# darskkaa/NTIRE-2026-Light-Field-Image-Super-Resolution-Challenge---Track-2-Efficiency

Measured on AMD Instinct MI355X. Metric: 5x5 x4-SR LF patches/sec (32^2->128^2), DistgSSR inference, higher is better.
Workload: dtype f32 (EPI branch stage 1 / 2 and fuse.0: fp32 operands as three exact bf16 terms on the bf16 MFMA pipe, six products, fp32 accumulation -- error against fp64 not above the fp32-MFMA kernels', tests/test_gpu_b3_accuracy.py; 3x3 convs, angular branch, init, head: fp32 MFMA)

## Files before the change

ntire-2026-light-field-image-super-resolution-challenge---track-2-efficiency_amd/csrc/distg_tail.hip:

```cpp
#include "lfsr_internal.h"

namespace {

typedef float f32x4t __attribute__((ext_vector_type(4)));
typedef unsigned u32x4t __attribute__((ext_vector_type(4)));

constexpr int DT_WAVES = 8;
constexpr int DT_FPLANE = 64 * 160;
constexpr int DT_FBYTES = 3 * DT_FPLANE * 2;
constexpr int DT_ESLOTS = 3 * 4 * 160;
constexpr int DT_EBYTES = DT_ESLOTS * 16;
constexpr int DT_AFLOATS = 25 * 16 * 16;
constexpr int DT_ABYTES = DT_AFLOATS * 4;
constexpr int DT_CROW = 84;
constexpr int DT_CBYTES = DT_WAVES * 16 * DT_CROW * 4;
constexpr int DT_SMEM = DT_FBYTES + DT_EBYTES + DT_ABYTES + DT_CBYTES;

struct DistgTailArgs {
  const float* S; int s_stride; int s_choff; int s_bytes;
  const float* TA; int ta_bytes;
  const float* TH; const float* TV; int te_bytes;
  const float* WA2;
  const uint4* WE2p;
  const float* WF;
  float* Y; int y_stride; int y_choff; int y_bytes;
  int B, H, W;
  float slope;
};

__device__ __forceinline__ void dt_split8(const f32x4t lo, const f32x4t hi, u32x4t& p0, u32x4t& p1, u32x4t& p2) {
  const float a[8] = {lo.x, lo.y, lo.z, lo.w, hi.x, hi.y, hi.z, hi.w};
#pragma unroll
  for (int j = 0; j < 4; ++j) { unsigned t0, t1, t2; lfsr_split_pair(a[2 * j], a[2 * j + 1], t0, t1, t2); p0[j] = t0; p1[j] = t1; p2[j] = t2; }
}

__device__ __forceinline__ void dt_mfma(f32x4t& c, const u32x4t a, const u32x4t b) {
  asm volatile("v_mfma_f32_16x16x32_bf16 %0, %1, %2, %0" : "+v"(c) : "v"(a), "v"(b));
}

__device__ __forceinline__ void dt_six2(f32x4t& c0, const u32x4t (&a)[3], const u32x4t (&x)[3], f32x4t& c1, const u32x4t (&b)[3], const u32x4t (&y)[3]) {
  dt_mfma(c0, a[2], x[0]); dt_mfma(c1, b[2], y[0]);
  dt_mfma(c0, a[0], x[2]); dt_mfma(c1, b[0], y[2]);
  dt_mfma(c0, a[1], x[1]); dt_mfma(c1, b[1], y[1]);
  dt_mfma(c0, a[1], x[0]); dt_mfma(c1, b[1], y[0]);
  dt_mfma(c0, a[0], x[1]); dt_mfma(c1, b[0], y[1]);
  dt_mfma(c0, a[0], x[0]); dt_mfma(c1, b[0], y[0]);
}

__global__ __launch_bounds__(512) void k_distg_tail(DistgTailArgs p) {
  extern __shared__ __attribute__((aligned(16))) unsigned char smem_raw[];
  unsigned short* const sF = reinterpret_cast<unsigned short*>(smem_raw);
  unsigned char* const sE = smem_raw + DT_FBYTES;
  float* const sA = reinterpret_cast<float*>(smem_raw + DT_FBYTES + DT_EBYTES);
  float* const sC = reinterpret_cast<float*>(smem_raw + DT_FBYTES + DT_EBYTES + DT_ABYTES);
  constexpr int A = 5, AA = 25;
  constexpr int EOOB = (int)0x80000000u;
  const int tid = threadIdx.x, lane = tid & 63, wave = tid >> 6;
  const int l15 = lane & 15, g = lane >> 4;
  const int HW = p.H * p.W, M = p.B * HW;
  const int ntiles = (M + 15) / 16;

  for (int i = tid; i < 64 * 20; i += 512) {
    const int r = i / 20, c = i - r * 20;
    const bool ok = c * 8 < 144;
    const float* src = p.WF + r * 144 + (ok ? c * 8 : 0);
    f32x4t lo = *reinterpret_cast<const f32x4t*>(src), hi = *reinterpret_cast<const f32x4t*>(src + 4);
    if (!ok) { lo = f32x4t{0.f, 0.f, 0.f, 0.f}; hi = lo; }
    u32x4t w0, w1, w2;
    dt_split8(lo, hi, w0, w1, w2);
    const int slot = (c * 64 + r) * 8;
    *reinterpret_cast<u32x4t*>(sF + 0 * DT_FPLANE + slot) = w0;
    *reinterpret_cast<u32x4t*>(sF + 1 * DT_FPLANE + slot) = w1;
    *reinterpret_cast<u32x4t*>(sF + 2 * DT_FPLANE + slot) = w2;
  }
  for (int i = tid; i < DT_ESLOTS; i += 512) reinterpret_cast<uint4*>(sE)[i] = p.WE2p[i];
  for (int i = tid; i < DT_AFLOATS / 4; i += 512) reinterpret_cast<float4*>(sA)[i] = reinterpret_cast<const float4*>(p.WA2)[i];
  __syncthreads();

  const __amdgpu_buffer_rsrc_t rsS = __builtin_amdgcn_make_buffer_rsrc(const_cast<float*>(p.S), 0, p.s_bytes, 0x00020000);
  const __amdgpu_buffer_rsrc_t rsA = __builtin_amdgcn_make_buffer_rsrc(const_cast<float*>(p.TA), 0, p.ta_bytes, 0x00020000);
  const __amdgpu_buffer_rsrc_t rsH = __builtin_amdgcn_make_buffer_rsrc(const_cast<float*>(p.TH), 0, p.te_bytes, 0x00020000);
  const __amdgpu_buffer_rsrc_t rsV = __builtin_amdgcn_make_buffer_rsrc(const_cast<float*>(p.TV), 0, p.te_bytes, 0x00020000);
  const __amdgpu_buffer_rsrc_t rsY = __builtin_amdgcn_make_buffer_rsrc(p.Y, 0, p.y_bytes, 0x00020000);
  float* const st = sC + wave * 16 * DT_CROW;
  const unsigned char* const wE = sE + (g * 160 + l15) * 16;
  const unsigned short* const wF = sF + (g * 64 + l15) * 8;
  const float* const bA = sA + l15 * 16 + 4 * g;

  for (int tile = (int)blockIdx.x * DT_WAVES + wave; tile < ntiles; tile += (int)gridDim.x * DT_WAVES) {
    const int m = tile * 16 + l15;
    const bool ok = m < M;
    const int mb = ok ? m / HW : 0, myx = ok ? m - mb * HW : 0;
    auto tro = [&](int q) { return ok ? (((mb * A + q) * HW + myx) * 32 + 4 * g) * 4 : EOOB; };
    auto pixo = [&](int view) { return ok ? ((mb * AA + view) * HW + myx) : -1; };
    const f32x4t a2 = __builtin_bit_cast(f32x4t, __builtin_amdgcn_raw_buffer_load_b128(rsA, ok ? (m * 16 + 4 * g) * 4 : EOOB, 0, 0));

    f32x4t sr0[2][2], sr1[2][2], vr0[2], vr1[2], hr[2];
    auto load_view = [&](int view, f32x4t (&sr)[2][2], f32x4t (&vr)[2]) {
      const int pix = pixo(view);
      const int so = pix >= 0 ? (pix * p.s_stride + p.s_choff + 8 * g) * 4 : EOOB;
#pragma unroll
      for (int s = 0; s < 2; ++s)
#pragma unroll
        for (int e = 0; e < 2; ++e) sr[s][e] = __builtin_bit_cast(f32x4t, __builtin_amdgcn_raw_buffer_load_b128(rsS, so == EOOB ? EOOB : so + (32 * s + 4 * e) * 4, 0, 0));
      const int vo = tro(view % A);
      vr[0] = __builtin_bit_cast(f32x4t, __builtin_amdgcn_raw_buffer_load_b128(rsV, vo, 0, 0));
      vr[1] = __builtin_bit_cast(f32x4t, __builtin_amdgcn_raw_buffer_load_b128(rsV, vo == EOOB ? EOOB : vo + 64, 0, 0));
    };
    auto load_h = [&](int u) {
      const int ho = tro(u);
      hr[0] = __builtin_bit_cast(f32x4t, __builtin_amdgcn_raw_buffer_load_b128(rsH, ho, 0, 0));
      hr[1] = __builtin_bit_cast(f32x4t, __builtin_amdgcn_raw_buffer_load_b128(rsH, ho == EOOB ? EOOB : ho + 64, 0, 0));
    };
    load_h(0);
    load_view(0, sr0, vr0);
    u32x4t hp[3];

    auto body = [&](int view, f32x4t (&sr)[2][2], f32x4t (&vr)[2], f32x4t (&srn)[2][2], f32x4t (&vrn)[2]) {
      const int u = view / A, v = view - A * u;
      if (view + 1 < AA) load_view(view + 1, srn, vrn);
      if (v == 0) dt_split8(hr[0], hr[1], hp[0], hp[1], hp[2]);
      if (v == A - 1 && u + 1 < A) load_h(u + 1);

      {
        const float4 b = *reinterpret_cast<const float4*>(bA + view * 256);
        f32x4t o = {0.f, 0.f, 0.f, 0.f};
        o = __builtin_amdgcn_mfma_f32_16x16x4f32(a2.x, b.x, o, 0, 0, 0);
        o = __builtin_amdgcn_mfma_f32_16x16x4f32(a2.y, b.y, o, 0, 0, 0);
        o = __builtin_amdgcn_mfma_f32_16x16x4f32(a2.z, b.z, o, 0, 0, 0);
        o = __builtin_amdgcn_mfma_f32_16x16x4f32(a2.w, b.w, o, 0, 0, 0);
#pragma unroll
        for (int r = 0; r < 4; ++r) {
          float z = o[r];
          z = z >= 0.f ? z : z * p.slope;
          st[(4 * g + r) * DT_CROW + l15] = z;
        }
      }

      {
        u32x4t vp[3];
        dt_split8(vr[0], vr[1], vp[0], vp[1], vp[2]);
        asm volatile("s_nop 4" : "+v"(hp[0]), "+v"(hp[1]), "+v"(hp[2]), "+v"(vp[0]), "+v"(vp[1]), "+v"(vp[2]));
        f32x4t e[2][2];
#pragma unroll
        for (int i = 0; i < 2; ++i) { e[i][0] = f32x4t{0.f, 0.f, 0.f, 0.f}; e[i][1] = e[i][0]; }
        asm volatile("s_nop 1" : "+v"(e[0][0]), "+v"(e[0][1]), "+v"(e[1][0]), "+v"(e[1][1]));
#pragma unroll
        for (int h = 0; h < 2; ++h) {
          u32x4t aH[3], aV[3];
#pragma unroll
          for (int pl = 0; pl < 3; ++pl) {
            aH[pl] = *reinterpret_cast<const u32x4t*>(wE + ((pl * 4) * 160 + 16 * (2 * v + h)) * 16);
            aV[pl] = *reinterpret_cast<const u32x4t*>(wE + ((pl * 4) * 160 + 16 * (2 * u + h)) * 16);
          }
          dt_six2(e[0][h], aH, hp, e[1][h], aV, vp);
        }
        asm volatile("s_nop 15\n\ts_nop 15" : "+v"(e[0][0]), "+v"(e[0][1]), "+v"(e[1][0]), "+v"(e[1][1]));
#pragma unroll
        for (int i = 0; i < 2; ++i)
#pragma unroll
          for (int h = 0; h < 2; ++h) {
            f32x4t z = e[i][h];
#pragma unroll
            for (int r = 0; r < 4; ++r) z[r] = fmaxf(z[r], z[r] * p.slope);
            *reinterpret_cast<f32x4t*>(st + l15 * DT_CROW + 16 + 32 * i + 16 * h + 4 * g) = z;
          }
      }
      __builtin_amdgcn_wave_barrier();

      u32x4t x0[5], x1[5], x2[5];
#pragma unroll
      for (int s = 0; s < 2; ++s) dt_split8(sr[s][0], sr[s][1], x0[s], x1[s], x2[s]);
#pragma unroll
      for (int s = 2; s < 5; ++s) {
        const float* cp = st + l15 * DT_CROW + 32 * (s - 2) + 8 * g;
        f32x4t lo = *reinterpret_cast<const f32x4t*>(cp), hi = *reinterpret_cast<const f32x4t*>(cp + 4);
        if (s == 4 && g >= 2) { lo = f32x4t{0.f, 0.f, 0.f, 0.f}; hi = lo; }
        dt_split8(lo, hi, x0[s], x1[s], x2[s]);
      }
      __builtin_amdgcn_wave_barrier();
      f32x4t acc[4];
#pragma unroll
      for (int t = 0; t < 4; ++t) acc[t] = f32x4t{0.f, 0.f, 0.f, 0.f};
#pragma unroll
      for (int s = 0; s < 5; ++s) asm volatile("s_nop 4" : "+v"(x0[s]), "+v"(x1[s]), "+v"(x2[s]));
      asm volatile("s_nop 1" : "+v"(acc[0]), "+v"(acc[1]), "+v"(acc[2]), "+v"(acc[3]));
#pragma unroll
      for (int s = 0; s < 5; ++s) {
        const u32x4t xs[3] = {x0[s], x1[s], x2[s]};
#pragma unroll
        for (int t = 0; t < 4; t += 2) {
          u32x4t wa[3], wb[3];
#pragma unroll
          for (int pl = 0; pl < 3; ++pl) {
            wa[pl] = *reinterpret_cast<const u32x4t*>(wF + pl * DT_FPLANE + (4 * s * 64 + t * 16) * 8);
            wb[pl] = *reinterpret_cast<const u32x4t*>(wF + pl * DT_FPLANE + (4 * s * 64 + (t + 1) * 16) * 8);
          }
          dt_six2(acc[t], wa, xs, acc[t + 1], wb, xs);
        }
      }
      asm volatile("s_nop 15\n\ts_nop 15" : "+v"(acc[0]), "+v"(acc[1]), "+v"(acc[2]), "+v"(acc[3]));
      const int pix = pixo(view);
      const int yo = pix >= 0 ? (pix * p.y_stride + p.y_choff + 4 * g) * 4 : EOOB;
#pragma unroll
      for (int t = 0; t < 4; ++t) {
        f32x4t z = acc[t];
#pragma unroll
        for (int r = 0; r < 4; ++r) z[r] = z[r] >= 0.f ? z[r] : z[r] * p.slope;
        __builtin_amdgcn_raw_buffer_store_b128(__builtin_bit_cast(u32x4t, z), rsY, yo == EOOB ? EOOB : yo + 64 * t, 0, 0);
        asm volatile("s_nop 1" : "+v"(z));
      }
    };
#pragma unroll 1
    for (int view = 0; view < AA - 1; view += 2) {
      body(view, sr0, vr0, sr1, vr1);
      body(view + 1, sr1, vr1, sr0, vr0);
    }
    body(AA - 1, sr0, vr0, sr1, vr1);
  }
}

}

int lfsr_distg_tail_launch(const float* spa, int spa_stride, int spa_choff, const float* t_a, const float* t_h, const float* t_v, const float* wa2_packed,
                           const float* we2_planes, const float* wf_packed, float* y, int y_stride, int y_choff, int B, int A, int h, int w, float slope,
                           hipStream_t st) {
  if (A != 5 || B <= 0 || h <= 0 || w <= 0 || !spa || !t_a || !t_h || !t_v || !wa2_packed || !we2_planes || !wf_packed || !y) return LFSR_E_ARG;
  if ((spa_stride | spa_choff | y_stride | y_choff) & 3 || spa_stride < spa_choff + 64 || y_stride < y_choff + 64) return LFSR_E_ARG;
  if (((uintptr_t)spa | (uintptr_t)t_a | (uintptr_t)t_h | (uintptr_t)t_v | (uintptr_t)wa2_packed | (uintptr_t)we2_planes | (uintptr_t)wf_packed | (uintptr_t)y) & 15)
    return LFSR_E_ARG;
  if (!(slope >= 0.f && slope <= 1.f)) return LFSR_E_ARG;
  const long long npix = (long long)B * A * A * h * w;
  if (npix * spa_stride * 4 >= (1LL << 31) || npix * y_stride * 4 >= (1LL << 31) || (long long)B * A * h * w * 32 * 4 >= (1LL << 31)) return LFSR_E_ARG;
  static std::atomic<bool> attr_set[64];
  static std::atomic<int> cus[64];
  int dev = 0;
  if (hipGetDevice(&dev) != hipSuccess || dev < 0 || dev >= 64) return LFSR_E_ARG;
  if (!attr_set[dev]) {
    hipError_t e = hipFuncSetAttribute(reinterpret_cast<const void*>(k_distg_tail), hipFuncAttributeMaxDynamicSharedMemorySize, DT_SMEM);
    if (e != hipSuccess) return LFSR_HIP_ERR(e);
    int v = 0;
    cus[dev] = (hipDeviceGetAttribute(&v, hipDeviceAttributeMultiprocessorCount, dev) == hipSuccess && v > 0) ? v : 256;
    attr_set[dev] = true;
  }
  DistgTailArgs p{};
  p.S = spa; p.s_stride = spa_stride; p.s_choff = spa_choff; p.s_bytes = (int)(npix * spa_stride * 4);
  p.TA = t_a; p.ta_bytes = (int)((long long)B * h * w * 16 * 4);
  p.TH = t_h; p.TV = t_v; p.te_bytes = (int)((long long)B * A * h * w * 32 * 4);
  p.WA2 = wa2_packed; p.WE2p = reinterpret_cast<const uint4*>(we2_planes); p.WF = wf_packed;
  p.Y = y; p.y_stride = y_stride; p.y_choff = y_choff; p.y_bytes = (int)(npix * y_stride * 4);
  p.B = B; p.H = h; p.W = w; p.slope = slope;
  const long long ntiles = ((long long)B * h * w + 15) / 16;
  long long grid = (ntiles + DT_WAVES - 1) / DT_WAVES;
  if (grid > cus[dev]) grid = cus[dev];
  hipLaunchKernelGGL(k_distg_tail, dim3((unsigned)grid), dim3(DT_WAVES * 64), DT_SMEM, st, p);
  LFSR_CHECK_LAUNCH();
  return LFSR_OK;
}

bool lfsr_distg_tail_ok(int A, int h, int w, const float* x, int x_stride, int x_choff, const float* t_h, const float* t_v) {
  if (A != 5 || h <= 0 || w <= 0 || h > 32 || w > 32 || !lfsr_ang_fused_ok(A) || !lfsr_epi_use_b3()) return false;
  const char* rsel = lfsr_sel("LFSR_ROWGEMM");
  const char* asel = lfsr_sel("LFSR_ANG");
  if ((rsel && (rsel[0] == 'f' || rsel[0] == '1')) || lfsr_sel("LFSR_NO_ROWGEMM") || (asel && asel[0] == 'g')) return false;
  if ((x_stride | x_choff) & 3 || x_stride < x_choff + 64 || (((uintptr_t)x | (uintptr_t)t_h | (uintptr_t)t_v) & 15)) return false;
  return true;
}

extern "C" int lfsr_distg_branch_tail_fwd(const float* x, int x_stride, int x_choff, const float* spa, int spa_stride, int spa_choff,
                                          const float* w_ang0, const float* w_ang2, const float* w_epi0, const float* w_epi2, const float* w_fuse0,
                                          float* t_a, float* t_h, float* t_v, float* y, int y_stride, int y_choff, int B, int A, int h, int w, float slope,
                                          void* stream) {
  LfsrOpTimer op_t("distg_tail", B, h * w, lfsr_stream(stream));
  if (!x || !spa || !w_ang0 || !w_ang2 || !w_epi0 || !w_epi2 || !w_fuse0 || !t_a || !t_h || !t_v || !y || B <= 0) return LFSR_E_ARG;
  if (!lfsr_distg_tail_ok(A, h, w, x, x_stride, x_choff, t_h, t_v)) return LFSR_E_ARG;
  if ((spa_stride | spa_choff | y_stride | y_choff) & 3 || spa_stride < spa_choff + 64 || y_stride < y_choff + 64) return LFSR_E_ARG;
  if (((uintptr_t)spa | (uintptr_t)t_a | (uintptr_t)w_ang2 | (uintptr_t)w_epi0 | (uintptr_t)w_epi2 | (uintptr_t)w_fuse0 | (uintptr_t)y) & 15) return LFSR_E_ARG;
  if (!(slope >= 0.f && slope <= 1.f)) return LFSR_E_ARG;
  const long long npix = (long long)B * A * A * h * w;
  if (npix * x_stride * 4 >= (1LL << 31) || npix * spa_stride * 4 >= (1LL << 31) || npix * y_stride * 4 >= (1LL << 31)) return LFSR_E_ARG;
  hipStream_t st = lfsr_stream(stream);
  int rc = lfsr_ang_fused_launch(x, x_stride, x_choff, w_ang0, nullptr, t_a, nullptr, 0, 0, B, A, h, w, slope, st);
  if (!rc) rc = lfsr_epi_b3_launch(x, x_stride, x_choff, w_epi0 + 25 * 32 * 64 + LFSR_EPI_WINO_FLOATS, nullptr, nullptr, 0, 0, 0, t_h, t_v, B, A, h, w, 3, slope, st);
  if (!rc) rc = lfsr_distg_tail_launch(spa, spa_stride, spa_choff, t_a, t_h, t_v, w_ang2, w_epi2 + 160 * 32, w_fuse0, y, y_stride, y_choff, B, A, h, w, slope, st);
  return rc;
}
```

Before: 2109.

## Prefetch first tile before weight staging, keep fuse weights in registers, zero-init MFMAs

New measurement: 2129 (median of 6 runs). About the same (+1.0%).

```diff
diff --git a/ntire-2026-light-field-image-super-resolution-challenge---track-2-efficiency_amd/csrc/distg_tail.hip b/ntire-2026-light-field-image-super-resolution-challenge---track-2-efficiency_amd/csrc/distg_tail.hip
--- a/ntire-2026-light-field-image-super-resolution-challenge---track-2-efficiency_amd/csrc/distg_tail.hip
+++ b/ntire-2026-light-field-image-super-resolution-challenge---track-2-efficiency_amd/csrc/distg_tail.hip
@@ -37,9 +37,14 @@
 __device__ __forceinline__ void dt_mfma(f32x4t& c, const u32x4t a, const u32x4t b) {
   asm volatile("v_mfma_f32_16x16x32_bf16 %0, %1, %2, %0" : "+v"(c) : "v"(a), "v"(b));
 }
-
+__device__ __forceinline__ void dt_mfma0(f32x4t& c, const u32x4t a, const u32x4t b) {
+  asm volatile("v_mfma_f32_16x16x32_bf16 %0, %1, %2, 0" : "=&v"(c) : "v"(a), "v"(b));
+}
+
+template <bool FIRST>
 __device__ __forceinline__ void dt_six2(f32x4t& c0, const u32x4t (&a)[3], const u32x4t (&x)[3], f32x4t& c1, const u32x4t (&b)[3], const u32x4t (&y)[3]) {
-  dt_mfma(c0, a[2], x[0]); dt_mfma(c1, b[2], y[0]);
+  if (FIRST) { dt_mfma0(c0, a[2], x[0]); dt_mfma0(c1, b[2], y[0]); }
+  else { dt_mfma(c0, a[2], x[0]); dt_mfma(c1, b[2], y[0]); }
   dt_mfma(c0, a[0], x[2]); dt_mfma(c1, b[0], y[2]);
   dt_mfma(c0, a[1], x[1]); dt_mfma(c1, b[1], y[1]);
   dt_mfma(c0, a[1], x[0]); dt_mfma(c1, b[1], y[0]);
@@ -54,11 +59,50 @@
   float* const sA = reinterpret_cast<float*>(smem_raw + DT_FBYTES + DT_EBYTES);
   float* const sC = reinterpret_cast<float*>(smem_raw + DT_FBYTES + DT_EBYTES + DT_ABYTES);
   constexpr int A = 5, AA = 25;
-  constexpr int EOOB = (int)0x80000000u;
+  constexpr unsigned EOOB = 0x80000000u;
   const int tid = threadIdx.x, lane = tid & 63, wave = tid >> 6;
   const int l15 = lane & 15, g = lane >> 4;
   const int HW = p.H * p.W, M = p.B * HW;
   const int ntiles = (M + 15) / 16;
+  const int tstride = (int)gridDim.x * DT_WAVES;
+
+  const __amdgpu_buffer_rsrc_t rsS = __builtin_amdgcn_make_buffer_rsrc(const_cast<float*>(p.S), 0, p.s_bytes, 0x00020000);
+  const __amdgpu_buffer_rsrc_t rsA = __builtin_amdgcn_make_buffer_rsrc(const_cast<float*>(p.TA), 0, p.ta_bytes, 0x00020000);
+  const __amdgpu_buffer_rsrc_t rsH = __builtin_amdgcn_make_buffer_rsrc(const_cast<float*>(p.TH), 0, p.te_bytes, 0x00020000);
+  const __amdgpu_buffer_rsrc_t rsV = __builtin_amdgcn_make_buffer_rsrc(const_cast<float*>(p.TV), 0, p.te_bytes, 0x00020000);
+  const __amdgpu_buffer_rsrc_t rsY = __builtin_amdgcn_make_buffer_rsrc(p.Y, 0, p.y_bytes, 0x00020000);
+  const unsigned sview = (unsigned)(HW * p.s_stride * 4), yview = (unsigned)(HW * p.y_stride * 4), tview = (unsigned)(HW * 32 * 4);
+
+  unsigned sbase = EOOB, ybase = EOOB, tbase = EOOB;
+  f32x4t a2;
+  f32x4t sr0[2][2], sr1[2][2], vr0[2], vr1[2], hr0[2], hr1[2];
+  auto load_view = [&](int view, f32x4t (&sr)[2][2], f32x4t (&vr)[2], f32x4t (&hr)[2]) {
+    const unsigned so = sbase + (unsigned)view * sview;
+#pragma unroll
+    for (int s = 0; s < 2; ++s)
+#pragma unroll
+      for (int e = 0; e < 2; ++e) sr[s][e] = __builtin_bit_cast(f32x4t, __builtin_amdgcn_raw_buffer_load_b128(rsS, so + (32 * s + 4 * e) * 4, 0, 0));
+    const unsigned vo = tbase + (unsigned)(view % A) * tview;
+    vr[0] = __builtin_bit_cast(f32x4t, __builtin_amdgcn_raw_buffer_load_b128(rsV, vo, 0, 0));
+    vr[1] = __builtin_bit_cast(f32x4t, __builtin_amdgcn_raw_buffer_load_b128(rsV, vo + 64, 0, 0));
+    const unsigned ho = tbase + (unsigned)(view / A) * tview;
+    hr[0] = __builtin_bit_cast(f32x4t, __builtin_amdgcn_raw_buffer_load_b128(rsH, ho, 0, 0));
+    hr[1] = __builtin_bit_cast(f32x4t, __builtin_amdgcn_raw_buffer_load_b128(rsH, ho + 64, 0, 0));
+  };
+  auto start_tile = [&](int tile) {
+    const int m = tile * 16 + l15;
+    const bool ok = m < M;
+    const int mb = ok ? m / HW : 0, myx = ok ? m - mb * HW : 0;
+    const int pix0 = mb * AA * HW + myx;
+    sbase = ok ? (unsigned)((pix0 * p.s_stride + p.s_choff + 8 * g) * 4) : EOOB;
+    ybase = ok ? (unsigned)((pix0 * p.y_stride + p.y_choff + 4 * g) * 4) : EOOB;
+    tbase = ok ? (unsigned)(((mb * A * HW + myx) * 32 + 4 * g) * 4) : EOOB;
+    a2 = __builtin_bit_cast(f32x4t, __builtin_amdgcn_raw_buffer_load_b128(rsA, ok ? (unsigned)((m * 16 + 4 * g) * 4) : EOOB, 0, 0));
+    load_view(0, sr0, vr0, hr0);
+  };
+
+  int tile = (int)blockIdx.x * DT_WAVES + wave;
+  if (tile < ntiles) start_tile(tile);
 
   for (int i = tid; i < 64 * 20; i += 512) {
     const int r = i / 20, c = i - r * 20;
@@ -77,50 +121,24 @@
   for (int i = tid; i < DT_AFLOATS / 4; i += 512) reinterpret_cast<float4*>(sA)[i] = reinterpret_cast<const float4*>(p.WA2)[i];
   __syncthreads();
 
-  const __amdgpu_buffer_rsrc_t rsS = __builtin_amdgcn_make_buffer_rsrc(const_cast<float*>(p.S), 0, p.s_bytes, 0x00020000);
-  const __amdgpu_buffer_rsrc_t rsA = __builtin_amdgcn_make_buffer_rsrc(const_cast<float*>(p.TA), 0, p.ta_bytes, 0x00020000);
-  const __amdgpu_buffer_rsrc_t rsH = __builtin_amdgcn_make_buffer_rsrc(const_cast<float*>(p.TH), 0, p.te_bytes, 0x00020000);
-  const __amdgpu_buffer_rsrc_t rsV = __builtin_amdgcn_make_buffer_rsrc(const_cast<float*>(p.TV), 0, p.te_bytes, 0x00020000);
-  const __amdgpu_buffer_rsrc_t rsY = __builtin_amdgcn_make_buffer_rsrc(p.Y, 0, p.y_bytes, 0x00020000);
   float* const st = sC + wave * 16 * DT_CROW;
   const unsigned char* const wE = sE + (g * 160 + l15) * 16;
   const unsigned short* const wF = sF + (g * 64 + l15) * 8;
+  auto wld = [&](int s, int t, int pl) { return *reinterpret_cast<const u32x4t*>(wF + pl * DT_FPLANE + (4 * s * 64 + t * 16) * 8); };
+  constexpr int DT_WKEEP = 24;
+  u32x4t wkeep[DT_WKEEP];
+#pragma unroll
+  for (int i = 0; i < DT_WKEEP; ++i) wkeep[i] = wld(i / 12, (i % 12) / 3, i % 3);
+  auto wop = [&](int s, int t, int pl) { const int i = s * 12 + t * 3 + pl; return i < DT_WKEEP ? wkeep[i] : wld(s, t, pl); };
   const float* const bA = sA + l15 * 16 + 4 * g;
 
-  for (int tile = (int)blockIdx.x * DT_WAVES + wave; tile < ntiles; tile += (int)gridDim.x * DT_WAVES) {
-    const int m = tile * 16 + l15;
-    const bool ok = m < M;
-    const int mb = ok ? m / HW : 0, myx = ok ? m - mb * HW : 0;
-    auto tro = [&](int q) { return ok ? (((mb * A + q) * HW + myx) * 32 + 4 * g) * 4 : EOOB; };
-    auto pixo = [&](int view) { return ok ? ((mb * AA + view) * HW + myx) : -1; };
-    const f32x4t a2 = __builtin_bit_cast(f32x4t, __builtin_amdgcn_raw_buffer_load_b128(rsA, ok ? (m * 16 + 4 * g) * 4 : EOOB, 0, 0));
-
-    f32x4t sr0[2][2], sr1[2][2], vr0[2], vr1[2], hr[2];
-    auto load_view = [&](int view, f32x4t (&sr)[2][2], f32x4t (&vr)[2]) {
-      const int pix = pixo(view);
-      const int so = pix >= 0 ? (pix * p.s_stride + p.s_choff + 8 * g) * 4 : EOOB;
-#pragma unroll
-      for (int s = 0; s < 2; ++s)
-#pragma unroll
-        for (int e = 0; e < 2; ++e) sr[s][e] = __builtin_bit_cast(f32x4t, __builtin_amdgcn_raw_buffer_load_b128(rsS, so == EOOB ? EOOB : so + (32 * s + 4 * e) * 4, 0, 0));
-      const int vo = tro(view % A);
-      vr[0] = __builtin_bit_cast(f32x4t, __builtin_amdgcn_raw_buffer_load_b128(rsV, vo, 0, 0));
-      vr[1] = __builtin_bit_cast(f32x4t, __builtin_amdgcn_raw_buffer_load_b128(rsV, vo == EOOB ? EOOB : vo + 64, 0, 0));
-    };
-    auto load_h = [&](int u) {
-      const int ho = tro(u);
-      hr[0] = __builtin_bit_cast(f32x4t, __builtin_amdgcn_raw_buffer_load_b128(rsH, ho, 0, 0));
-      hr[1] = __builtin_bit_cast(f32x4t, __builtin_amdgcn_raw_buffer_load_b128(rsH, ho == EOOB ? EOOB : ho + 64, 0, 0));
-    };
-    load_h(0);
-    load_view(0, sr0, vr0);
+  for (; tile < ntiles; tile += tstride) {
     u32x4t hp[3];
 
-    auto body = [&](int view, f32x4t (&sr)[2][2], f32x4t (&vr)[2], f32x4t (&srn)[2][2], f32x4t (&vrn)[2]) {
+    auto body = [&](int view, f32x4t (&sr)[2][2], f32x4t (&vr)[2], f32x4t (&hr)[2], f32x4t (&srn)[2][2], f32x4t (&vrn)[2], f32x4t (&hrn)[2]) {
       const int u = view / A, v = view - A * u;
-      if (view + 1 < AA) load_view(view + 1, srn, vrn);
+      load_view(view + 1 < AA ? view + 1 : view, srn, vrn, hrn);
       if (v == 0) dt_split8(hr[0], hr[1], hp[0], hp[1], hp[2]);
-      if (v == A - 1 && u + 1 < A) load_h(u + 1);
 
       {
         const float4 b = *reinterpret_cast<const float4*>(bA + view * 256);
@@ -130,11 +148,7 @@
         o = __builtin_amdgcn_mfma_f32_16x16x4f32(a2.z, b.z, o, 0, 0, 0);
         o = __builtin_amdgcn_mfma_f32_16x16x4f32(a2.w, b.w, o, 0, 0, 0);
 #pragma unroll
-        for (int r = 0; r < 4; ++r) {
-          float z = o[r];
-          z = z >= 0.f ? z : z * p.slope;
-          st[(4 * g + r) * DT_CROW + l15] = z;
-        }
+        for (int r = 0; r < 4; ++r) st[(4 * g + r) * DT_CROW + l15] = fmaxf(o[r], o[r] * p.slope);
       }
 
       {
@@ -143,9 +157,6 @@
         asm volatile("s_nop 4" : "+v"(hp[0]), "+v"(hp[1]), "+v"(hp[2]), "+v"(vp[0]), "+v"(vp[1]), "+v"(vp[2]));
         f32x4t e[2][2];
 #pragma unroll
-        for (int i = 0; i < 2; ++i) { e[i][0] = f32x4t{0.f, 0.f, 0.f, 0.f}; e[i][1] = e[i][0]; }
-        asm volatile("s_nop 1" : "+v"(e[0][0]), "+v"(e[0][1]), "+v"(e[1][0]), "+v"(e[1][1]));
-#pragma unroll
         for (int h = 0; h < 2; ++h) {
           u32x4t aH[3], aV[3];
 #pragma unroll
@@ -153,7 +164,7 @@
             aH[pl] = *reinterpret_cast<const u32x4t*>(wE + ((pl * 4) * 160 + 16 * (2 * v + h)) * 16);
             aV[pl] = *reinterpret_cast<const u32x4t*>(wE + ((pl * 4) * 160 + 16 * (2 * u + h)) * 16);
           }
-          dt_six2(e[0][h], aH, hp, e[1][h], aV, vp);
+          dt_six2<true>(e[0][h], aH, hp, e[1][h], aV, vp);
         }
         asm volatile("s_nop 15\n\ts_nop 15" : "+v"(e[0][0]), "+v"(e[0][1]), "+v"(e[1][0]), "+v"(e[1][1]));
 #pragma unroll
@@ -181,10 +192,7 @@
       __builtin_amdgcn_wave_barrier();
       f32x4t acc[4];
 #pragma unroll
-      for (int t = 0; t < 4; ++t) acc[t] = f32x4t{0.f, 0.f, 0.f, 0.f};
-#pragma unroll
       for (int s = 0; s < 5; ++s) asm volatile("s_nop 4" : "+v"(x0[s]), "+v"(x1[s]), "+v"(x2[s]));
-      asm volatile("s_nop 1" : "+v"(acc[0]), "+v"(acc[1]), "+v"(acc[2]), "+v"(acc[3]));
 #pragma unroll
       for (int s = 0; s < 5; ++s) {
         const u32x4t xs[3] = {x0[s], x1[s], x2[s]};
@@ -193,30 +201,31 @@
           u32x4t wa[3], wb[3];
 #pragma unroll
           for (int pl = 0; pl < 3; ++pl) {
-            wa[pl] = *reinterpret_cast<const u32x4t*>(wF + pl * DT_FPLANE + (4 * s * 64 + t * 16) * 8);
-            wb[pl] = *reinterpret_cast<const u32x4t*>(wF + pl * DT_FPLANE + (4 * s * 64 + (t + 1) * 16) * 8);
+            wa[pl] = wop(s, t, pl);
+            wb[pl] = wop(s, t + 1, pl);
           }
-          dt_six2(acc[t], wa, xs, acc[t + 1], wb, xs);
+          if (s == 0) dt_six2<true>(acc[t], wa, xs, acc[t + 1], wb, xs);
+          else dt_six2<false>(acc[t], wa, xs, acc[t + 1], wb, xs);
         }
       }
       asm volatile("s_nop 15\n\ts_nop 15" : "+v"(acc[0]), "+v"(acc[1]), "+v"(acc[2]), "+v"(acc[3]));
-      const int pix = pixo(view);
-      const int yo = pix >= 0 ? (pix * p.y_stride + p.y_choff + 4 * g) * 4 : EOOB;
+      const unsigned yo = ybase + (unsigned)view * yview;
 #pragma unroll
       for (int t = 0; t < 4; ++t) {
         f32x4t z = acc[t];
 #pragma unroll
-        for (int r = 0; r < 4; ++r) z[r] = z[r] >= 0.f ? z[r] : z[r] * p.slope;
-        __builtin_amdgcn_raw_buffer_store_b128(__builtin_bit_cast(u32x4t, z), rsY, yo == EOOB ? EOOB : yo + 64 * t, 0, 0);
+        for (int r = 0; r < 4; ++r) z[r] = fmaxf(z[r], z[r] * p.slope);
+        __builtin_amdgcn_raw_buffer_store_b128(__builtin_bit_cast(u32x4t, z), rsY, yo + 64 * t, 0, 0);
         asm volatile("s_nop 1" : "+v"(z));
       }
     };
+    body(0, sr0, vr0, hr0, sr1, vr1, hr1);
 #pragma unroll 1
-    for (int view = 0; view < AA - 1; view += 2) {
-      body(view, sr0, vr0, sr1, vr1);
-      body(view + 1, sr1, vr1, sr0, vr0);
+    for (int view = 1; view < AA; view += 2) {
+      body(view, sr1, vr1, hr1, sr0, vr0, hr0);
+      body(view + 1, sr0, vr0, hr0, sr1, vr1, hr1);
     }
-    body(AA - 1, sr0, vr0, sr1, vr1);
+    if (tile + tstride < ntiles) start_tile(tile + tstride);
   }
 }
 
```
